# sulaimanvesal/PointCloudUDA

Hardware: AMD Instinct MI355X
Metric: adversarial train-step images/sec (seg+3 discr) at 256x256 (higher is better)
Workload: dtype bf16x3 MFMA (split-bf16, fp32 accumulate; fp32 storage); 1 GPU; MS-CMRSeg full UDA: UNet(PointNet head) + d1 + d2 + d4, 256x256x1, 4 classes; per_gpu_batch=32, global_batch=32, precision=bf16x3, parallelism=dp1, ranks_in_group=1, collective=none, streams=discriminators concurrent, d_target_forward=replayed from the adversarial pass of the same step, launch=eager (256 host cores for this rank)

## Files before the change

include/pcuda_hip.h:

```cpp
#ifndef PCUDA_HIP_H
#define PCUDA_HIP_H

#include <stddef.h>
#include <stdint.h>

#ifdef __cplusplus
extern "C" {
#endif

#define PCUDA_OK 0
#define PCUDA_E_BADARG (-1)
#define PCUDA_E_UNSUPPORTED (-2)
#define PCUDA_E_LAUNCH (-3)
#define PCUDA_E_WORKSPACE (-4)

#define PCUDA_PREC_BF16X3 0
#define PCUDA_PREC_BF16 1

typedef void* pcuda_stream_t;

#define PCUDA_ABI_VERSION 5
int pcuda_version(void);
size_t pcuda_abi_struct_size(int which);
int pcuda_device_count(void);
// ... 2 lines not shown
long long pcuda_launch_count(int reset);
long long pcuda_fallback_count(void);
const char* pcuda_last_kernel(void);
int pcuda_clock_probe(unsigned long long* out2_dev, float* sink_dev, int iters, pcuda_stream_t s);

#define PCUDA_FAM_CONV_FWD 0
#define PCUDA_FAM_CONV_WGRAD 1
#define PCUDA_FAM_POINTWISE 2
#define PCUDA_FAM_DENSE_F32 3
#define PCUDA_FAM_COUNT 4
int pcuda_prof_enable(int on);
int pcuda_prof_reset(void);
int pcuda_prof_read(int family, double* ms, double* work, long long* launches);
int pcuda_prof_dump(const char* path);
int pcuda_debug_read_clocks(unsigned long long* out8);

typedef struct pcuda_conv_geom {
  int n;
  int cin, cout;
  int in_h, in_w;
  int out_h, out_w;
  int k, stride, pad, dil;
  int in_up;
} pcuda_conv_geom;

typedef struct pcuda_src {
  const float* p1; long long sn1, sc1; const float* scale1; const float* shift1;
  const float* p2; long long sn2, sc2; const float* scale2; const float* shift2;
  int c1;
} pcuda_src;
typedef struct pcuda_dst {
  float* p1; long long sn1, sc1;
  float* p2; long long sn2, sc2;
  int c1;
} pcuda_dst;

size_t pcuda_conv2d_packed_fwd_bytes(const pcuda_conv_geom* g, int prec);
size_t pcuda_conv2d_packed_dgrad_bytes(const pcuda_conv_geom* g, int prec);
int pcuda_conv2d_pack_fwd(const pcuda_conv_geom* g, int prec, const float* w, void* packed, pcuda_stream_t s);
int pcuda_conv2d_pack_dgrad(const pcuda_conv_geom* g, int prec, const float* w, void* packed, pcuda_stream_t s);
int pcuda_conv2d_pack_all(const pcuda_conv_geom* g, int prec, const float* w, void* packed_fwd, void* packed_dgrad,
                          pcuda_stream_t s);
size_t pcuda_conv2d_pack_job_bytes(void);
int pcuda_conv2d_pack_jobs_fill(const pcuda_conv_geom* g, int prec, const float* w, void* packed_fwd, void* packed_dgrad,
                                void* host_jobs, int max_jobs, int* job_blocks);
int pcuda_conv2d_pack_table(const void* dev_jobs, const int* dev_first_block, int njobs, int total_blocks, pcuda_stream_t s);

int pcuda_conv2d_d1_forward_ok(const pcuda_conv_geom* g);
int pcuda_conv2d_fwd_tiles(const pcuda_conv_geom* g, int prec);
int pcuda_conv2d_forward(const pcuda_conv_geom* g, int prec, const pcuda_src* x, const void* packed_w,
                         const float* bias, float slope, const pcuda_dst* y, float* bn_partials,
                         pcuda_stream_t s);
int pcuda_conv2d_dgrad(const pcuda_conv_geom* g, int prec, const pcuda_src* dy, const void* packed_w_dgrad,
                       const pcuda_dst* dx, int accumulate, pcuda_stream_t s);
int pcuda_conv2d_dgrad_tiles(const pcuda_conv_geom* g, int prec);
int pcuda_conv2d_dgrad_bnred(const pcuda_conv_geom* g, int prec, const pcuda_src* dy, const void* packed_w_dgrad,
                             const pcuda_dst* dx, int accumulate, const float* a, long long a_sn, long long a_sc,
                             const float* mean, const float* invstd, float* red_partials, pcuda_stream_t s);
int pcuda_conv2d_dgrad_lrelu(const pcuda_conv_geom* g, int prec, const pcuda_src* dy, const void* packed_w_dgrad,
                             const pcuda_dst* dx, const float* a, long long a_sn, long long a_sc, float slope,
                             pcuda_stream_t s);
int pcuda_conv2d_dgrad_fold(const pcuda_conv_geom* g, int prec, const pcuda_src* dy, const void* packed_w_dgrad,
                            const pcuda_dst* dx_half, const float* a, long long a_sn, long long a_sc, const float* mean,
                            const float* invstd, float* red_partials, pcuda_stream_t s);
size_t pcuda_conv2d_wgrad_workspace_size(const pcuda_conv_geom* g);
int pcuda_conv2d_wgrad(const pcuda_conv_geom* g, int prec, const pcuda_src* x, const float* dy,
                       long long dy_sn, long long dy_sc, float* dw, float* db, int accumulate,
                       void* workspace, size_t workspace_bytes, pcuda_stream_t s);

#define PCUDA_REDUCE_MAX_JOBS 56
typedef struct {
  const float* partial;
  long long numel;
  float* dw;
  const float* db_partial;
  long long nb;
  float* db;
  int ksplit, nkg, accumulate, ntaps;
} pcuda_reduce_job;
int pcuda_conv2d_wgrad_partial(const pcuda_conv_geom* g, int prec, const pcuda_src* x, const float* dy,
                               long long dy_sn, long long dy_sc, float* dw, float* db, int accumulate,
                               void* workspace, size_t workspace_bytes, pcuda_reduce_job* job, pcuda_stream_t s);
int pcuda_wgrad_reduce_batch(const pcuda_reduce_job* host_jobs, int njobs, pcuda_stream_t s);

int pcuda_bn_finalize(const float* partials, int ntiles, int c, long long count, const float* gamma,
                      const float* beta, float eps, float momentum, float* running_mean, float* running_var,
                      float* mean, float* invstd, float* scale, float* shift, pcuda_stream_t s);
int pcuda_bn_stats(const float* a, long long sn, long long sc, int n, int c, long long hw,
                   float* partials, int* ntiles, pcuda_stream_t s);
#define PCUDA_BN_APPLY_RELU 1
#define PCUDA_BN_APPLY_FMA 2
int pcuda_bn_apply(const float* a, long long a_sn, long long a_sc, const float* scale, const float* shift,
                   int flags, float* y, long long y_sn, long long y_sc, int n, int c, long long hw,
                   pcuda_stream_t s);
int pcuda_bn_bwd_reduce(const float* dy, long long dy_sn, long long dy_sc, const float* dy2, long long dy2_sn,
                        long long dy2_sc, const float* a, long long a_sn, long long a_sc, const float* mean,
                        const float* invstd, const float* scale, const float* shift, int post_relu, int n, int c,
                        long long hw, float* red, int* ntiles, pcuda_stream_t s);
int pcuda_bn_bwd_finalize(const float* red, int ntiles, int c, long long count, const float* gamma,
                          const float* invstd, const float* mean, float* dgamma, float* dbeta, int accumulate,
                          float* coef , pcuda_stream_t s);
int pcuda_bn_bwd_apply(const float* dy, long long dy_sn, long long dy_sc, const float* dy2, long long dy2_sn,
                       long long dy2_sc, const float* a, long long a_sn, long long a_sc, const float* coef,
                       const float* scale, const float* shift, int post_relu, float act_slope, float* dz,
                       long long dz_sn, long long dz_sc, int n, int c, long long hw, pcuda_stream_t s);
int pcuda_lrelu_bwd(const float* dy, long long dy_sn, long long dy_sc, const float* dy2, long long dy2_sn,
                    long long dy2_sc, const float* a, long long a_sn, long long a_sc, float slope, float* dz,
                    long long dz_sn, long long dz_sc, int n, int c, long long hw, pcuda_stream_t s);
int pcuda_channel_sum(const float* dz, long long sn, long long sc, int n, int c, long long hw, float* db,
                      int accumulate, float* workspace, size_t workspace_bytes, pcuda_stream_t s);

int pcuda_maxpool2_fwd(const float* x, long long x_sn, long long x_sc, const float* scale, const float* shift,
                       float* y, long long y_sn, long long y_sc, uint8_t* idx, int n, int c, int h, int w,
                       pcuda_stream_t s);
int pcuda_maxpool2_bwd(const float* dy, long long dy_sn, long long dy_sc, const float* dy2, long long dy2_sn,
                       long long dy2_sc, const uint8_t* idx, float* dx, long long dx_sn, long long dx_sc,
                       int accumulate, int n, int c, int h, int w, pcuda_stream_t s);
typedef struct pcuda_pooled {
  const float* g; long long g_sn, g_sc;
  const float* g2; long long g2_sn, g2_sc;
  const uint8_t* idx;
  int h, w;
} pcuda_pooled;
int pcuda_bn_bwd_reduce_pooled(const pcuda_pooled* pool, const float* dy, long long dy_sn, long long dy_sc, const float* a,
                               long long a_sn, long long a_sc, const float* mean, const float* invstd, int n, int c,
                               float* red, int* ntiles, pcuda_stream_t s);
int pcuda_bn_bwd_apply_pooled(const pcuda_pooled* pool, const float* dy, long long dy_sn, long long dy_sc, const float* a,
                              long long a_sn, long long a_sc, const float* coef, float act_slope, float* dz, long long dz_sn,
                              long long dz_sc, int n, int c, pcuda_stream_t s);
int pcuda_lrelu_bwd_pooled(const pcuda_pooled* pool, const float* dy, long long dy_sn, long long dy_sc, const float* a,
                           long long a_sn, long long a_sc, float slope, float* dz, long long dz_sn, long long dz_sc, int n,
                           int c, pcuda_stream_t s);
int pcuda_upsample2_bwd(const float* dy, long long dy_sn, long long dy_sc, float* dx, long long dx_sn,
                        long long dx_sc, int accumulate, int n, int c, int h, int w, pcuda_stream_t s);
int pcuda_upsample2_bwd_bnred(const float* dy, long long dy_sn, long long dy_sc, float* dx, long long dx_sn,
                              long long dx_sc, int accumulate, const float* a, long long a_sn, long long a_sc,
                              const float* mean, const float* invstd, float* red, int* ntiles, int n, int c, int h, int w,
                              pcuda_stream_t s);
int pcuda_bilinear_fwd(const float* x, long long x_sn, long long x_sc, int n, int c, int h, int w, float* y, int oh,
                       int ow, pcuda_stream_t s);
int pcuda_bilinear_bwd(const float* dy, int n, int c, int oh, int ow, float* dx, long long dx_sn, long long dx_sc,
                       int h, int w, pcuda_stream_t s);
int pcuda_unfold_taps(const float* x, long long x_sn, long long x_sc, int n, int c, int h, int w, int k, int stride,
                      int pad, int dil, float* u, int oh, int ow, pcuda_stream_t s);
int pcuda_add4(const float* a, const float* b, const float* c, const float* d, float* y, long long numel,
               pcuda_stream_t s);
int pcuda_mul(const float* a, const float* b, float* y, long long numel, pcuda_stream_t s);

#define PCUDA_ACT_SIGMOID 0
#define PCUDA_ACT_SOFTMAX 1
int pcuda_entropy_fwd(const float* logits, int mode, float norm, float* ent, float* prob, int n, int c,
                      long long hw, pcuda_stream_t s);
int pcuda_entropy_bwd(const float* logits, int mode, float norm, const float* dent, const float* dprob,
                      float* dlogits, int accumulate, int n, int c, long long hw, pcuda_stream_t s);
int pcuda_entropy_bwd2(const float* logits, int mode, float norm, const float* dent, const float* dprob, const float* dmean,
                       float* dlogits, int accumulate, int n, int c, long long hw, pcuda_stream_t s);
size_t pcuda_sum_all_workspace_size(void);
int pcuda_sum_all(const float* x, long long numel, double scale, float* out, void* workspace, size_t workspace_bytes,
                  pcuda_stream_t s);
size_t pcuda_seg_loss_workspace_size(int n, int c, long long hw);
int pcuda_seg_loss_fwd(const float* logits, const uint8_t* onehot, int mode, int n, int c, long long hw,
                       float* out2, void* workspace, size_t workspace_bytes, pcuda_stream_t s);
int pcuda_seg_loss_bwd(const float* logits, const uint8_t* onehot, int mode, int n, int c, long long hw,
                       const float* g_main, const float* g_jac, float* dlogits, const void* workspace,
                       pcuda_stream_t s);
int pcuda_bce_const_fwd(const float* x, long long numel, float label, float* loss, float* acc, pcuda_stream_t s);
// ... 251 lines not shown
```

pointcloududa_amd/_lib.py:

```python
from __future__ import annotations

import ctypes as C
import os

_HERE = os.path.dirname(os.path.abspath(__file__))
LIB_PATH = os.environ.get("PCUDA_LIB") or os.path.join(_HERE, "lib", "libpcuda_hip.so")

PREC_BF16X3, PREC_BF16 = 0, 1
ACT_SIGMOID, ACT_SOFTMAX = 0, 1
OV_DICE_CLASS, OV_DICE_SAMPLE = 1, 2
FAM_CONV_FWD, FAM_CONV_WGRAD, FAM_POINTWISE, FAM_DENSE_F32 = 0, 1, 2, 3

c_f32p = C.c_void_p
i32, i64, f32, f64, vp, sz = C.c_int, C.c_longlong, C.c_float, C.c_double, C.c_void_p, C.c_size_t


class ConvGeom(C.Structure):
    _fields_ = [("n", i32), ("cin", i32), ("cout", i32), ("in_h", i32), ("in_w", i32), ("out_h", i32),
                ("out_w", i32), ("k", i32), ("stride", i32), ("pad", i32), ("dil", i32), ("in_up", i32)]


class ReduceJob(C.Structure):
    _fields_ = [("partial", C.c_void_p), ("numel", C.c_longlong), ("dw", C.c_void_p), ("db_partial", C.c_void_p),
                ("nb", C.c_longlong), ("db", C.c_void_p), ("ksplit", C.c_int), ("nkg", C.c_int), ("accumulate", C.c_int),
                ("ntaps", C.c_int)]


class Src(C.Structure):
    _fields_ = [("p1", vp), ("sn1", i64), ("sc1", i64), ("scale1", vp), ("shift1", vp),
                ("p2", vp), ("sn2", i64), ("sc2", i64), ("scale2", vp), ("shift2", vp), ("c1", i32)]


class Dst(C.Structure):
    _fields_ = [("p1", vp), ("sn1", i64), ("sc1", i64), ("p2", vp), ("sn2", i64), ("sc2", i64), ("c1", i32)]


class Pooled(C.Structure):
    _fields_ = [("g", vp), ("g_sn", i64), ("g_sc", i64), ("g2", vp), ("g2_sn", i64), ("g2_sc", i64), ("idx", vp),
                ("h", i32), ("w", i32)]


_PROTOS = {
    "pcuda_version": (i32, []),
    "pcuda_device_count": (i32, []),
    "pcuda_last_error": (C.c_char_p, []),
    "pcuda_build_hash": (C.c_char_p, []),
    "pcuda_launch_count": (i64, [i32]),
    "pcuda_fallback_count": (i64, []),
    "pcuda_abi_struct_size": (sz, [i32]),
    "pcuda_last_kernel": (C.c_char_p, []),
    "pcuda_clock_probe": (i32, [vp, vp, i32, vp]),
    "pcuda_prof_enable": (i32, [i32]),
    "pcuda_prof_reset": (i32, []),
    "pcuda_prof_read": (i32, [i32, C.POINTER(C.c_double), C.POINTER(C.c_double), C.POINTER(i64)]),
    "pcuda_prof_dump": (i32, [C.c_char_p]),
    "pcuda_debug_read_clocks": (i32, [vp]),
    "pcuda_conv2d_packed_fwd_bytes": (sz, [C.POINTER(ConvGeom), i32]),
    "pcuda_conv2d_packed_dgrad_bytes": (sz, [C.POINTER(ConvGeom), i32]),
    "pcuda_conv2d_pack_fwd": (i32, [C.POINTER(ConvGeom), i32, vp, vp, vp]),
    "pcuda_conv2d_pack_all": (i32, [C.POINTER(ConvGeom), i32, vp, vp, vp, vp]),
    "pcuda_conv2d_pack_dgrad": (i32, [C.POINTER(ConvGeom), i32, vp, vp, vp]),
    "pcuda_conv2d_pack_job_bytes": (sz, []),
    "pcuda_conv2d_pack_jobs_fill": (i32, [C.POINTER(ConvGeom), i32, vp, vp, vp, vp, i32, C.POINTER(i32)]),
    "pcuda_conv2d_pack_table": (i32, [vp, vp, i32, i32, vp]),
    "pcuda_conv2d_fwd_tiles": (i32, [C.POINTER(ConvGeom), i32]),
    "pcuda_conv2d_forward": (i32, [C.POINTER(ConvGeom), i32, C.POINTER(Src), vp, vp, f32, C.POINTER(Dst), vp, vp]),
    "pcuda_conv2d_d1_forward_ok": (i32, [C.POINTER(ConvGeom)]),
    "pcuda_conv2d_dgrad": (i32, [C.POINTER(ConvGeom), i32, C.POINTER(Src), vp, C.POINTER(Dst), i32, vp]),
    "pcuda_conv2d_dgrad_tiles": (i32, [C.POINTER(ConvGeom), i32]),
    "pcuda_conv2d_dgrad_bnred": (i32, [C.POINTER(ConvGeom), i32, C.POINTER(Src), vp, C.POINTER(Dst), i32, vp, i64, i64, vp,
                                       vp, vp, vp]),
    "pcuda_conv2d_dgrad_fold": (i32, [C.POINTER(ConvGeom), i32, C.POINTER(Src), vp, C.POINTER(Dst), vp, i64, i64, vp, vp, vp, vp]),
    "pcuda_conv2d_dgrad_lrelu": (i32, [C.POINTER(ConvGeom), i32, C.POINTER(Src), vp, C.POINTER(Dst), vp, i64, i64, f32, vp]),
    "pcuda_conv2d_wgrad_workspace_size": (sz, [C.POINTER(ConvGeom)]),
    "pcuda_conv2d_wgrad": (i32, [C.POINTER(ConvGeom), i32, C.POINTER(Src), vp, i64, i64, vp, vp, i32, vp, sz, vp]),
    "pcuda_conv2d_wgrad_partial": (i32, [C.POINTER(ConvGeom), i32, C.POINTER(Src), vp, i64, i64, vp, vp, i32, vp, sz,
                                         C.POINTER(ReduceJob), vp]),
    "pcuda_wgrad_reduce_batch": (i32, [C.POINTER(ReduceJob), i32, vp]),
    "pcuda_bn_finalize": (i32, [vp, i32, i32, i64, vp, vp, f32, f32, vp, vp, vp, vp, vp, vp, vp]),
    "pcuda_bn_stats": (i32, [vp, i64, i64, i32, i32, i64, vp, C.POINTER(i32), vp]),
    "pcuda_bn_apply": (i32, [vp, i64, i64, vp, vp, i32, vp, i64, i64, i32, i32, i64, vp]),
    "pcuda_bn_bwd_reduce": (i32, [vp, i64, i64, vp, i64, i64, vp, i64, i64, vp, vp, vp, vp, i32, i32, i32, i64, vp,
                                  C.POINTER(i32), vp]),
    "pcuda_bn_bwd_finalize": (i32, [vp, i32, i32, i64, vp, vp, vp, vp, vp, i32, vp, vp]),
    "pcuda_bn_bwd_apply": (i32, [vp, i64, i64, vp, i64, i64, vp, i64, i64, vp, vp, vp, i32, f32, vp, i64, i64, i32,
                                 i32, i64, vp]),
    "pcuda_lrelu_bwd": (i32, [vp, i64, i64, vp, i64, i64, vp, i64, i64, f32, vp, i64, i64, i32, i32, i64, vp]),
    "pcuda_channel_sum": (i32, [vp, i64, i64, i32, i32, i64, vp, i32, vp, sz, vp]),
    "pcuda_maxpool2_fwd": (i32, [vp, i64, i64, vp, vp, vp, i64, i64, vp, i32, i32, i32, i32, vp]),
    "pcuda_maxpool2_bwd": (i32, [vp, i64, i64, vp, i64, i64, vp, vp, i64, i64, i32, i32, i32, i32, i32, vp]),
    "pcuda_bn_bwd_reduce_pooled": (i32, [C.POINTER(Pooled), vp, i64, i64, vp, i64, i64, vp, vp, i32, i32, vp, C.POINTER(i32), vp]),
    "pcuda_bn_bwd_apply_pooled": (i32, [C.POINTER(Pooled), vp, i64, i64, vp, i64, i64, vp, f32, vp, i64, i64, i32, i32, vp]),
    "pcuda_lrelu_bwd_pooled": (i32, [C.POINTER(Pooled), vp, i64, i64, vp, i64, i64, f32, vp, i64, i64, i32, i32, vp]),
    "pcuda_upsample2_bwd": (i32, [vp, i64, i64, vp, i64, i64, i32, i32, i32, i32, i32, vp]),
    "pcuda_upsample2_bwd_bnred": (i32, [vp, i64, i64, vp, i64, i64, i32, vp, i64, i64, vp, vp, vp, C.POINTER(i32), i32, i32,
                                        i32, i32, vp]),
    "pcuda_bilinear_fwd": (i32, [vp, i64, i64, i32, i32, i32, i32, vp, i32, i32, vp]),
    "pcuda_bilinear_bwd": (i32, [vp, i32, i32, i32, i32, vp, i64, i64, i32, i32, vp]),
    "pcuda_unfold_taps": (i32, [vp, i64, i64, i32, i32, i32, i32, i32, i32, i32, i32, vp, i32, i32, vp]),
    "pcuda_add4": (i32, [vp, vp, vp, vp, vp, i64, vp]),
    "pcuda_mul": (i32, [vp, vp, vp, i64, vp]),
    "pcuda_entropy_fwd": (i32, [vp, i32, f32, vp, vp, i32, i32, i64, vp]),
    "pcuda_entropy_bwd": (i32, [vp, i32, f32, vp, vp, vp, i32, i32, i32, i64, vp]),
    "pcuda_entropy_bwd2": (i32, [vp, i32, f32, vp, vp, vp, vp, i32, i32, i32, i64, vp]),
    "pcuda_sum_all_workspace_size": (sz, []),
    "pcuda_sum_all": (i32, [vp, i64, C.c_double, vp, vp, sz, vp]),
    "pcuda_seg_loss_workspace_size": (sz, [i32, i32, i64]),
    "pcuda_seg_loss_fwd": (i32, [vp, vp, i32, i32, i32, i64, vp, vp, sz, vp]),
    "pcuda_seg_loss_bwd": (i32, [vp, vp, i32, i32, i32, i64, vp, vp, vp, vp, vp]),
    "pcuda_jaccard_workspace_size": (sz, [i32]),
    "pcuda_jaccard_fwd": (i32, [vp, vp, i32, i32, i32, i64, f32, vp, vp, sz, vp]),
    "pcuda_jaccard_bwd": (i32, [vp, i32, i32, i32, i64, f32, vp, vp, vp, vp]),
    "pcuda_seg_loss_ov_workspace_size": (sz, [i32, i32, i64, i32]),
    "pcuda_seg_loss_ov_fwd": (i32, [vp, vp, i32, i32, C.c_double, i32, i32, i64, vp, vp, sz, vp]),
    "pcuda_seg_loss_ov_bwd": (i32, [vp, vp, i32, i32, i32, i32, i64, vp, vp, vp, vp, sz, vp]),
    "pcuda_dice_workspace_size": (sz, [i32, i32, i64, i32]),
    "pcuda_dice_fwd": (i32, [vp, vp, i32, i32, i32, i64, i32, f32, vp, vp, sz, vp]),
    "pcuda_dice_bwd": (i32, [vp, i32, i32, i32, i64, i32, vp, vp, vp, sz, vp]),
    "pcuda_dice_labels_workspace_size": (sz, [i32, i32, i64]),
    "pcuda_dice_labels_fwd": (i32, [vp, vp, i32, i32, i32, i64, f32, vp, vp, vp, sz, vp]),
    "pcuda_dice_labels_bwd": (i32, [vp, vp, i32, i32, i32, i64, vp, vp, vp, sz, vp]),
    "pcuda_bce_const_fwd": (i32, [vp, i64, f32, vp, vp, vp]),
    "pcuda_bce_const_bwd": (i32, [vp, i64, f32, vp, f32, vp, vp]),
    "pcuda_nn_loss_workspace_floats": (sz, [i32, i32]),
    "pcuda_nn_loss_fwd": (i32, [vp, vp, i32, i32, vp, vp, vp, vp]),
    "pcuda_nn_loss_bwd": (i32, [vp, vp, i32, i32, vp, vp, vp, vp, vp]),
    "pcuda_dice_metric": (i32, [vp, vp, i32, i32, i64, vp, vp, sz, vp]),
    "pcuda_assemble_batch": (i32, [vp, vp, i32, i32, i32, i32, i32, i32, vp, vp, vp]),
    "pcuda_minmax_workspace_size": (sz, []),
    "pcuda_minmax": (i32, [vp, i64, vp, vp, sz, vp]),
    "pcuda_augment_assemble": (i32, [vp, i32, vp, i32, i32, i32, i32, i32, i32, vp, vp, vp, i32, vp, vp, vp, vp, vp, vp, vp]),
    "pcuda_quantize_u8": (i32, [vp, i64, vp, vp, vp]),
    "pcuda_augment_assemble_dequant": (i32, [vp, vp, i32, i32, i32, i32, i32, i32, vp, vp, vp, vp, vp, vp, vp, vp, vp, vp]),
    "pcuda_photometric_workspace_size": (sz, [i32, i32, i32, i32]),
    "pcuda_photometric": (i32, [vp, vp, i32, i32, i32, i32, i32, vp, vp, vp, vp, vp, sz, vp]),
    "pcuda_geometric_workspace_size": (sz, [i32, i32, i32, i32, i32]),
    "pcuda_geometric": (i32, [vp, vp, vp, vp, i32, i32, i32, i32, i32, vp, vp, vp, vp, vp, sz, vp]),
    "pcuda_geometric_cubic": (i32, [vp, vp, vp, vp, i32, i32, i32, i32, i32, vp, vp, vp, vp, vp, sz, vp]),
    "pcuda_stylize_workspace_size": (sz, [i32, i32, i32, i32]),
    "pcuda_stylize": (i32, [vp, vp, i32, i32, i32, i32, i32, vp, vp, vp, vp, vp, vp, sz, vp]),
    "pcuda_stylize_connect_workspace_size": (sz, [i32, i32, i32, i32]),
    "pcuda_stylize_connect": (i32, [vp, vp, i32, i32, i32, i32, i32, vp, vp, vp, vp, vp, vp, sz, vp]),
    "pcuda_stylize_scaled_workspace_size": (sz, [i32, i32, i32, i32]),
    "pcuda_stylize_scaled": (i32, [vp, vp, i32, i32, i32, i32, i32, vp, vp, vp, vp, vp, vp, sz, vp]),
    "pcuda_crop_pad_workspace_size": (sz, [i32, i32, i32, i32]),
    "pcuda_crop_pad": (i32, [vp, vp, vp, vp, i32, i32, i32, i32, vp, vp, vp, sz, vp]),
    "pcuda_match_hist_workspace_size": (sz, [i32, i32, i32, i32, i32]),
    "pcuda_match_hist": (i32, [vp, vp, i32, i32, i32, i32, i32, vp, vp, vp, i32, vp, sz, vp]),
    "pcuda_hist_bank_size": (sz, [i32, i32, i32, i32, i32]),
    "pcuda_hist_bank_workspace_size": (sz, [i32, i32, i32, i32, i32]),
    "pcuda_hist_bank_build": (i32, [vp, i32, i32, i32, i32, i32, vp, sz, vp, vp, sz, vp]),
    "pcuda_match_hist_bank_workspace_size": (sz, [i32, i32, i32, i32, i32]),
    "pcuda_match_hist_bank": (i32, [vp, vp, i32, i32, i32, i32, i32, vp, i32, i32, i32, vp, vp, sz, vp]),
    "pcuda_fourier_bank_size": (sz, [i32, i32, i32]),
    "pcuda_fourier_bank_workspace_size": (sz, [i32, i32, i32, i32, i32]),
    "pcuda_fourier_bank_build": (i32, [vp, i32, i32, i32, i32, i32, i32, vp, sz, vp, sz, vp]),
    "pcuda_fourier_adapt_workspace_size": (sz, [i32, i32, i32, i32, i32]),
    "pcuda_fourier_adapt": (i32, [vp, vp, i32, i32, i32, i32, i32, vp, i32, i32, vp, vp, i32, f64, f64, vp, sz, vp]),
    "pcuda_clahe_workspace_size": (sz, [i32, i32, i32]),
    "pcuda_clahe": (i32, [vp, vp, i32, i32, i32, f64, i32, i32, i32, vp, sz, vp]),
    "pcuda_rescale_resize_crop_u8_workspace_size": (sz, []),
# ... 109 lines not shown
```

pointcloududa_amd/csrc/conv_wgrad.hip:

```cpp
#include "conv_igemm.h"
#include "conv_host.h"

struct ReduceJobs {
  int n;
  int first_block[PCUDA_REDUCE_MAX_JOBS + 1];
  pcuda_reduce_job j[PCUDA_REDUCE_MAX_JOBS];
};

__global__ __launch_bounds__(1024) void wgrad_reduce_batch_kernel(const ReduceJobs jobs) {
  __shared__ float sh[16][64];
  int lo = 0, hi = jobs.n - 1;
  while (lo < hi) {
    const int mid = (lo + hi + 1) >> 1;
    if (jobs.first_block[mid] <= (int)blockIdx.x) lo = mid; else hi = mid - 1;
  }
  const pcuda_reduce_job& jb = jobs.j[lo];
  const float* partial = jb.partial;
  long long numel = jb.numel;
  float* dw = jb.dw;
  int ntaps = jb.ntaps;
  const int ksplit = jb.ksplit, nkg = jb.nkg;
  const int lane = threadIdx.x & 63, kg = threadIdx.x >> 6;
  const long long nblk_w = (numel + 63) / 64;
  long long blk = (int)blockIdx.x - jobs.first_block[lo];
  if (blk >= nblk_w) { blk -= nblk_w; partial = jb.db_partial; numel = jb.nb; dw = jb.db; ntaps = 1; }
  const long long i = blk * 64 + lane;
  float s = 0.f;
  if (i < numel && kg < nkg) {
    int k = kg;
    for (; k + 7 * nkg < ksplit; k += 8 * nkg) {
      float v[8];
#pragma unroll
      for (int u = 0; u < 8; ++u) v[u] = partial[(long long)(k + u * nkg) * numel + i];
#pragma unroll
      for (int u = 0; u < 8; ++u) s += v[u];
    }
    for (; k < ksplit; k += nkg) s += partial[(long long)k * numel + i];
  }
  sh[kg][lane] = s;
  __syncthreads();
  if (kg == 0 && i < numel) {
    float t = 0.f;
    for (int q = 0; q < nkg; ++q) t += sh[q][lane];
    long long o = i;
    if (ntaps > 1) {
      const long long cc = numel / ntaps;
      const long long tt = i / cc, r = i - tt * cc;
      o = r * ntaps + tt;
    }
    dw[o] = jb.accumulate ? dw[o] + t : t;
  }
}

static int reduce_blocks(const pcuda_reduce_job& jb) { return cdiv(jb.numel, 64) + (jb.db ? cdiv(jb.nb, 64) : 0); }

static int launch_reduce_jobs(const ReduceJobs& jobs, int threads, hipStream_t s) {
  hipLaunchKernelGGL(wgrad_reduce_batch_kernel, dim3(jobs.first_block[jobs.n]), dim3(threads), 0, s, jobs);
  PCUDA_CHECK_LAUNCH("wgrad_reduce_batch_kernel");
  return PCUDA_OK;
}

static pcuda_reduce_job reduce_job(const float* partial, long long numel, int ksplit, float* dw, int accumulate, int ntaps,
                                   const float* db_partial, long long nb, float* db) {
  pcuda_reduce_job jb;
  memset(&jb, 0, sizeof(jb));
  jb.partial = partial; jb.numel = numel; jb.ksplit = ksplit; jb.dw = dw; jb.accumulate = accumulate; jb.ntaps = ntaps;
  jb.db_partial = db_partial; jb.nb = db ? nb : 0; jb.db = db;
  jb.nkg = 1;
  while (jb.nkg < 16 && jb.nkg * 2 <= ksplit) jb.nkg <<= 1;
  return jb;
}

static int launch_reduce_job(const pcuda_reduce_job& jb, hipStream_t s) {
  ReduceJobs jobs;
  jobs.n = 1;
  jobs.j[0] = jb;
  jobs.first_block[0] = 0;
  jobs.first_block[1] = reduce_blocks(jb);
  return launch_reduce_jobs(jobs, 64 * jb.nkg, s);
}
int launch_wgrad_reduce(const float* partial, long long numel, int ksplit, float* dw, int accumulate, int ntaps,
                        const float* db_partial, long long nb, float* db, hipStream_t s) {
  return launch_reduce_job(reduce_job(partial, numel, ksplit, dw, accumulate, ntaps, db_partial, nb, db), s);
}

WgradSlabs wgrad_slabs(const WgradCall& c, int slices, int ntaps) {
  WgradSlabs sl;
  sl.welems = (long long)c.g->cout * c.g->cin * c.g->k * c.g->k;
  sl.partial = (float*)c.workspace;
  sl.db_partial = c.db ? sl.partial + (size_t)slices * sl.welems : nullptr;
  sl.slices = slices; sl.ntaps = ntaps;
  return sl;
}

int wgrad_finish(const WgradCall& c, const WgradSlabs& sl) {
  const pcuda_reduce_job jb = reduce_job(sl.partial, sl.welems, sl.slices, c.dw, c.accumulate, sl.ntaps, sl.db_partial, c.g->cout, c.db);
  if (!c.defer) return launch_reduce_job(jb, c.s);
  *c.defer = jb;
  return PCUDA_OK;
}

extern "C" int pcuda_wgrad_reduce_batch(const pcuda_reduce_job* host_jobs, int njobs, pcuda_stream_t s) {
  if (!host_jobs || njobs < 0) PCUDA_FAIL(PCUDA_E_BADARG, "wgrad_reduce_batch: bad arguments");
  int done = 0;
  while (done < njobs) {
    ReduceJobs jobs;
    jobs.n = 0;
    int blocks = 0;
    for (; done < njobs && jobs.n < PCUDA_REDUCE_MAX_JOBS; ++done) {
      const pcuda_reduce_job& jb = host_jobs[done];
      if (jb.ksplit <= 0) continue;
      if (!jb.partial || !jb.dw || jb.numel <= 0 || jb.nkg < 1 || jb.nkg > 16 || (jb.db && !jb.db_partial))
        PCUDA_FAIL(PCUDA_E_BADARG, "wgrad_reduce_batch: bad job %d", done);
      jobs.first_block[jobs.n] = blocks;
      jobs.j[jobs.n++] = jb;
      blocks += reduce_blocks(jb);
    }
    if (jobs.n == 0) break;
    jobs.first_block[jobs.n] = blocks;
    ProfScope prof(PCUDA_FAM_POINTWISE, 0.0, (hipStream_t)s, "wgrad reduce batch");
    const int rc = launch_reduce_jobs(jobs, 1024, (hipStream_t)s);
    if (rc) return rc;
  }
  return PCUDA_OK;
}

namespace {

struct WgradPlan {
  int co_blks, co_tile, n_co_tiles, n_chunks, tap_groups, taps_per_group, tw, th, tiles_x, tiles_y, ksplit;
  int ih_t, iw_t;
};

struct TileSpan {
  long long halo, clipped;
};
TileSpan tile_span(const pcuda_conv_geom* g, long long ih, long long iw) {
  return {ih * iw, (ih < g->in_h ? ih : g->in_h) * (iw < g->in_w ? iw : g->in_w) + 1};
}
size_t stage_lds(long long x_pixels, int co_tile, size_t mul) {
  return (size_t)x_pixels * IG_REC_BYTES * mul + (size_t)co_tile * WG_ZROW * mul;
}

struct WgradStage {
  bool clamp;
  int x_cap;
  size_t lds;
};
WgradStage wgrad_stage(const WgradPlan& w, const pcuda_conv_geom* g, size_t mul) {
  const TileSpan t = tile_span(g, w.ih_t, w.iw_t);
  WgradStage st;
  st.clamp = t.clipped * 2 <= t.halo || stage_lds(t.halo, w.co_tile, mul) > (size_t)LDS_HARD;
  st.x_cap = (int)(st.clamp ? t.clipped : t.halo);
  st.lds = stage_lds(st.x_cap, w.co_tile, mul);
  return st;
}

WgradPlan plan_wgrad(const pcuda_conv_geom* g) {
  WgradPlan w;
  w.co_blks = ig_co_blks(g->cout);
  w.co_tile = 32 * w.co_blks;
  w.n_co_tiles = cdiv(g->cout, w.co_tile);
  w.n_chunks = cdiv(g->cin, 32);
  const int ntaps = g->k * g->k;
  w.tap_groups = ntaps <= 16 ? 1 : cdiv(ntaps, 9);
  w.taps_per_group = cdiv(ntaps, w.tap_groups);
  const int span = (g->k - 1) * g->dil;
  {
    int cand[16];
    const int nc = tile_width_candidates(g->out_w, 128, cand);
    long long best_key = -1;
    w.tw = 32; w.th = 4;
    for (int ci = 0; ci < nc; ++ci) {
      const int tw = cand[ci], th = 128 / tw;
      if (th < 1) continue;
      const TileSpan t = tile_span(g, (th - 1) * g->stride + span + 1, (tw - 1) * g->stride + span + 1);
      const long long cap = t.halo < t.clipped ? t.halo : t.clipped;
      if (stage_lds(cap, w.co_tile, 2) > (size_t)LDS_HARD) continue;
      const long long staged = (t.clipped * 2 <= t.halo) ? t.clipped : t.halo;
      const long long key = ((long long)cdiv(g->out_w, tw) * cdiv(g->out_h, th) << 24) + (staged > 768 ? (1ll << 22) : 0) +
                            ((tw & 31) ? (1ll << 20) : 0) + t.halo;
      if (best_key < 0 || key < best_key) { best_key = key; w.tw = tw; w.th = th; }
    }
  }
  const int TW = w.tw, TH = w.th;
  w.tiles_x = cdiv(g->out_w, TW);
  w.tiles_y = cdiv(g->out_h, TH);
  w.ih_t = (TH - 1) * g->stride + span + 1;
  w.iw_t = (TW - 1) * g->stride + span + 1;
  const long long ntiles = (long long)g->n * w.tiles_x * w.tiles_y;
  const int base = w.n_co_tiles * w.n_chunks * w.tap_groups;
  static const int tgt32 = env_knob("PCUDA_WG_BLOCKS32", 768);
  static const int tgt64 = env_knob("PCUDA_WG_BLOCKS64", 1024);
  static const int tgt1 = env_knob("PCUDA_WG_BLOCKS1", 256);
  const bool one_per_cu = wgrad_stage(w, g, 2).lds > (size_t)LDS_HARD / 2;
  long long ks = (one_per_cu ? tgt1 : (w.co_blks == 1 ? tgt32 : tgt64)) / base;
  if (ks < 1) ks = 1;
  if (ks > ntiles) ks = ntiles;
  const long long welems = (long long)g->cout * g->cin * ntaps;
  while (ks > 1 && ks * welems * 4 > (64ll << 20)) ks >>= 1;
  if (ks >= 8) ks &= ~7ll;
  w.ksplit = (int)ks;
  return w;
}

int wgrad_prefetch(const WgradCall& c, const WgradPlan& w, int x_cap) {
// ... 133 lines not shown
```

pointcloududa_amd/csrc/dense.hip:

```cpp
#include "common.h"

struct GemmParams {
  const float* a; long long a_sb, a_si, a_sl;
  const float* b; long long b_sb, b_sl, b_sj;
  float* c; long long c_sb, c_si, c_sj;
  const float* bias;
  int m, n, k, accumulate;
};

#define GT 32
__global__ __launch_bounds__(256) void gemm_kernel(const GemmParams p) {
  __shared__ float As[GT][GT + 1], Bs[GT][GT + 1];
  const int bz = blockIdx.z;
  const float* A = p.a + bz * p.a_sb;
  const float* B = p.b + bz * p.b_sb;
  float* C = p.c + bz * p.c_sb;
  const int i0 = blockIdx.y * GT, j0 = blockIdx.x * GT;
  const int tj = threadIdx.x & 31, ti = threadIdx.x >> 5;
  float acc[4] = {0.f, 0.f, 0.f, 0.f};
  for (int l0 = 0; l0 < p.k; l0 += GT) {
    for (int e = threadIdx.x; e < GT * GT; e += 256) {
      const int r = e >> 5, cc = e & 31;
      int ia, la;
      if (p.a_sl == 1) { ia = r; la = cc; } else { ia = cc; la = r; }
      As[ia][la] = (i0 + ia < p.m && l0 + la < p.k) ? A[(i0 + ia) * p.a_si + (l0 + la) * p.a_sl] : 0.f;
      int lb, jb;
      if (p.b_sj == 1) { lb = r; jb = cc; } else { lb = cc; jb = r; }
      Bs[lb][jb] = (l0 + lb < p.k && j0 + jb < p.n) ? B[(l0 + lb) * p.b_sl + (j0 + jb) * p.b_sj] : 0.f;
    }
    __syncthreads();
#pragma unroll 8
    for (int l = 0; l < GT; ++l) {
      const float bv = Bs[l][tj];
#pragma unroll
      for (int q = 0; q < 4; ++q) acc[q] += As[ti * 4 + q][l] * bv;
    }
    __syncthreads();
  }
  const int j = j0 + tj;
  if (j < p.n) {
    const float bj = p.bias ? p.bias[j] : 0.f;
#pragma unroll
    for (int q = 0; q < 4; ++q) {
      const int i = i0 + ti * 4 + q;
      if (i < p.m) {
        float* dst = C + i * p.c_si + j * p.c_sj;
        const float v = acc[q] + bj;
        *dst = p.accumulate ? *dst + v : v;
      }
    }
  }
}

#define SK_COLS 8
#define SK_WAVES 16
__global__ __launch_bounds__(64 * SK_WAVES) void gemm_skinny_kernel(const GemmParams p) {
  __shared__ float red[SK_WAVES][64][SK_COLS];
  const int lane = threadIdx.x & 63, wv = threadIdx.x >> 6;
  const int j0 = blockIdx.x * SK_COLS;
  const int i = min(lane, p.m - 1);
  const float* arow = p.a + (long long)i * p.a_si;
  const int kq = (p.k + SK_WAVES - 1) / SK_WAVES, l_lo = wv * kq, l_hi = min(p.k, l_lo + kq);
  float acc[SK_COLS];
#pragma unroll
  for (int c = 0; c < SK_COLS; ++c) acc[c] = 0.f;
  const float* bcol[SK_COLS];
#pragma unroll
  for (int c = 0; c < SK_COLS; ++c) bcol[c] = p.b + (long long)min(j0 + c, p.n - 1) * p.b_sj;
#pragma unroll 4
  for (int l = l_lo; l < l_hi; ++l) {
    const float av = arow[(long long)l * p.a_sl];
#pragma unroll
    for (int c = 0; c < SK_COLS; ++c) acc[c] = fmaf(av, bcol[c][(long long)l * p.b_sl], acc[c]);
  }
#pragma unroll
  for (int c = 0; c < SK_COLS; ++c) red[wv][lane][c] = acc[c];
  __syncthreads();
  for (int e = threadIdx.x; e < 64 * SK_COLS; e += 64 * SK_WAVES) {
    const int r = e / SK_COLS, c = e - r * SK_COLS, j = j0 + c;
    if (r < p.m && j < p.n) {
      float v = 0.f;
#pragma unroll
      for (int q = 0; q < SK_WAVES; ++q) v += red[q][r][c];
      v += p.bias ? p.bias[j] : 0.f;
      float* dst = p.c + (long long)r * p.c_si + (long long)j * p.c_sj;
      *dst = p.accumulate ? *dst + v : v;
    }
  }
}


__global__ __launch_bounds__(256) void colsum_kernel(const float* __restrict__ dy, int m, int n, float* db,
                                                     int accumulate, int cp) {
  __shared__ float sh[256];
  const int rparts = 256 / cp;
  const int c = threadIdx.x % cp, rp = threadIdx.x / cp;
  const int j = blockIdx.x * cp + c;
  float s = 0.f;
  if (j < n)
    for (int i = rp; i < m; i += rparts) s += dy[(long long)i * n + j];
  sh[threadIdx.x] = s;
  __syncthreads();
  for (int half = rparts >> 1; half > 0; half >>= 1) {
    if (rp < half) sh[threadIdx.x] += sh[threadIdx.x + half * cp];
    __syncthreads();
  }
  if (rp == 0 && j < n) db[j] = accumulate ? db[j] + sh[c] : sh[c];
}

__global__ void splitk_reduce_kernel(const float* __restrict__ part, long long numel, int ksplit,
                                     float* __restrict__ out, int accumulate) {
  for (long long i = blockIdx.x * (long long)blockDim.x + threadIdx.x; i < numel;
       i += (long long)gridDim.x * blockDim.x) {
    float s = 0.f;
    for (int k = 0; k < ksplit; ++k) s += part[(long long)k * numel + i];
    out[i] = accumulate ? out[i] + s : s;
  }
}

__global__ __launch_bounds__(256) void max_points_fwd_kernel(const float* __restrict__ x, int rows, int l,
                                                             float* __restrict__ y, int* __restrict__ idx) {
  const int row = blockIdx.x * 4 + (threadIdx.x >> 6), lane = threadIdx.x & 63;
  if (row >= rows) return;
  const float* p = x + (long long)row * l;
  float best = -INFINITY;
  int bi = 0x7fffffff;
  for (int i = lane; i < l; i += 64) {
    const float v = p[i];
    if (v > best) { best = v; bi = i; }
  }
#pragma unroll
  for (int o = 32; o > 0; o >>= 1) {
    const float ov = __shfl_xor(best, o, 64);
    const int oi = __shfl_xor(bi, o, 64);
    if (ov > best || (ov == best && oi < bi)) { best = ov; bi = oi; }
  }
  if (lane == 0) { y[row] = best; idx[row] = bi; }
}

__global__ __launch_bounds__(256) void max_points_bwd_kernel(const float* __restrict__ dy, const int* __restrict__ idx,
                                                             int rows, int l, float* __restrict__ dx) {
  const long long total = (long long)rows * l;
  for (long long e = blockIdx.x * 256ll + threadIdx.x; e < total; e += 256ll * gridDim.x) {
    const int row = (int)(e / l), i = (int)(e - (long long)row * l);
    dx[e] = (idx[row] == i) ? dy[row] : 0.f;
  }
}

namespace {
int launch_gemm(const GemmParams& p, int batch, hipStream_t s) {
  if (p.m <= 0 || p.n <= 0 || p.k <= 0 || batch <= 0) PCUDA_FAIL(PCUDA_E_BADARG, "gemm: bad dims");
  if (batch == 1 && p.m <= 64 && p.k >= 64) {
    hipLaunchKernelGGL(gemm_skinny_kernel, dim3(cdiv(p.n, SK_COLS)), dim3(64 * SK_WAVES), 0, s, p);
    PCUDA_CHECK_LAUNCH("gemm_skinny_kernel");
    return PCUDA_OK;
  }
  dim3 grid(cdiv(p.n, GT), cdiv(p.m, GT), batch);
  hipLaunchKernelGGL(gemm_kernel, grid, dim3(256), 0, s, p);
  PCUDA_CHECK_LAUNCH("gemm_kernel");
  return PCUDA_OK;
}
}

extern "C" int pcuda_linear_fwd(const float* x, const float* w, const float* b, float* y, int m, int k, int n,
                                pcuda_stream_t s) {
  if (!x || !w || !y) PCUDA_FAIL(PCUDA_E_BADARG, "linear_fwd: null pointer");
  GemmParams p = {x, 0, k, 1, w, 0, 1, k, y, 0, n, 1, b, m, n, k, 0};
  return launch_gemm(p, 1, (hipStream_t)s);
}

extern "C" int pcuda_linear_bwd_x(const float* dy, const float* w, float* dx, int m, int k, int n, int accumulate,
                                  pcuda_stream_t s) {
  if (!dy || !w || !dx) PCUDA_FAIL(PCUDA_E_BADARG, "linear_bwd_x: null pointer");
  GemmParams p = {dy, 0, n, 1, w, 0, k, 1, dx, 0, k, 1, nullptr, m, k, n, accumulate};
  return launch_gemm(p, 1, (hipStream_t)s);
}

extern "C" size_t pcuda_linear_bwd_w_workspace_size(int m, int k, int n) {
  const long long out_elems = (long long)n * k;
  if (m >= 2048 && out_elems <= 65536) {
    int ks = m / 256;
    if (ks > 64) ks = 64;
    return (size_t)(ks + 1) * out_elems * sizeof(float);
  }
  return 0;
}

extern "C" int pcuda_linear_bwd_w(const float* dy, const float* x, float* dw, float* db, int m, int k, int n,
                                  int accumulate, void* workspace, size_t workspace_bytes, pcuda_stream_t s) {
  if (!dy || !x || !dw) PCUDA_FAIL(PCUDA_E_BADARG, "linear_bwd_w: null pointer");
  const long long out_elems = (long long)n * k;
  const size_t need = pcuda_linear_bwd_w_workspace_size(m, k, n);
  int rc;
  if (need > 0 && workspace && workspace_bytes >= need) {
    float* slab = (float*)workspace;
    int ks = m / 256;
    if (ks > 64) ks = 64;
    const int mk = (m + ks - 1) / ks;
    const int full = m / mk;
    GemmParams pb = {dy, (long long)mk * n, 1, n, x, (long long)mk * k, k, 1, slab, out_elems, k, 1, nullptr, n, k, mk, 0};
    rc = launch_gemm(pb, full, (hipStream_t)s);
    if (rc) return rc;
    int nsl = full;
    if (m - full * mk > 0) {
      GemmParams pt = {dy + (long long)full * mk * n, 0, 1, n, x + (long long)full * mk * k, 0, k, 1,
                       slab + (long long)full * out_elems, 0, k, 1, nullptr, n, k, m - full * mk, 0};
      rc = launch_gemm(pt, 1, (hipStream_t)s);
      if (rc) return rc;
      ++nsl;
    }
    hipLaunchKernelGGL(splitk_reduce_kernel, dim3(cdiv(out_elems, 256)), dim3(256), 0, (hipStream_t)s,
                       (const float*)slab, out_elems, nsl, dw, accumulate);
    PCUDA_CHECK_LAUNCH("splitk_reduce_kernel");
  } else {
    GemmParams p = {dy, 0, 1, n, x, 0, k, 1, dw, 0, k, 1, nullptr, n, k, m, accumulate};
    rc = launch_gemm(p, 1, (hipStream_t)s);
    if (rc) return rc;
  }
  if (db) {
    int cp = 1;
    while (cp < n && cp < 64) cp <<= 1;
    hipLaunchKernelGGL(colsum_kernel, dim3(cdiv(n, cp)), dim3(256), 0, (hipStream_t)s, dy, m, n, db, accumulate, cp);
    PCUDA_CHECK_LAUNCH("colsum_kernel");
  }
  return PCUDA_OK;
}

extern "C" int pcuda_bmm(const float* a, const float* bmat, float* c, int batch, int m, int k, int n, int ta, int tb,
                         int accumulate, pcuda_stream_t s) {
  if (!a || !bmat || !c) PCUDA_FAIL(PCUDA_E_BADARG, "bmm: null pointer");
  GemmParams p;
  p.a = a; p.a_sb = (long long)m * k; p.a_si = ta ? 1 : k; p.a_sl = ta ? m : 1;
  p.b = bmat; p.b_sb = (long long)k * n; p.b_sl = tb ? 1 : n; p.b_sj = tb ? k : 1;
  p.c = c; p.c_sb = (long long)m * n; p.c_si = n; p.c_sj = 1;
  p.bias = nullptr; p.m = m; p.n = n; p.k = k; p.accumulate = accumulate;
  return launch_gemm(p, batch, (hipStream_t)s);
}
// ... 18 lines not shown
```

Measured before the change: 786.8 img/s.

## Vectorize wgrad reduce, add LDS-staged skinny GEMM, unroll split-K reduce

```diff
diff --git a/include/pcuda_hip.h b/include/pcuda_hip.h
--- a/include/pcuda_hip.h
+++ b/include/pcuda_hip.h
@@ -108,6 +108,7 @@
                                long long dy_sn, long long dy_sc, float* dw, float* db, int accumulate,
                                void* workspace, size_t workspace_bytes, pcuda_reduce_job* job, pcuda_stream_t s);
 int pcuda_wgrad_reduce_batch(const pcuda_reduce_job* host_jobs, int njobs, pcuda_stream_t s);
+int pcuda_wgrad_reduce_bounds(const pcuda_reduce_job* job, long long* out4);
 
 int pcuda_bn_finalize(const float* partials, int ntiles, int c, long long count, const float* gamma,
                       const float* beta, float eps, float momentum, float* running_mean, float* running_var,
diff --git a/pointcloududa_amd/_lib.py b/pointcloududa_amd/_lib.py
--- a/pointcloududa_amd/_lib.py
+++ b/pointcloududa_amd/_lib.py
@@ -77,6 +77,7 @@
     "pcuda_conv2d_wgrad_partial": (i32, [C.POINTER(ConvGeom), i32, C.POINTER(Src), vp, i64, i64, vp, vp, i32, vp, sz,
                                          C.POINTER(ReduceJob), vp]),
     "pcuda_wgrad_reduce_batch": (i32, [C.POINTER(ReduceJob), i32, vp]),
+    "pcuda_wgrad_reduce_bounds": (i32, [C.POINTER(ReduceJob), C.POINTER(i64)]),
     "pcuda_bn_finalize": (i32, [vp, i32, i32, i64, vp, vp, f32, f32, vp, vp, vp, vp, vp, vp, vp]),
     "pcuda_bn_stats": (i32, [vp, i64, i64, i32, i32, i64, vp, C.POINTER(i32), vp]),
     "pcuda_bn_apply": (i32, [vp, i64, i64, vp, vp, i32, vp, i64, i64, i32, i32, i64, vp]),
diff --git a/pointcloududa_amd/csrc/conv_wgrad.hip b/pointcloududa_amd/csrc/conv_wgrad.hip
--- a/pointcloududa_amd/csrc/conv_wgrad.hip
+++ b/pointcloududa_amd/csrc/conv_wgrad.hip
@@ -1,5 +1,94 @@
 #include "conv_igemm.h"
 #include "conv_host.h"
+
+#ifndef PCUDA_REDUCE_FILL
+#define PCUDA_REDUCE_FILL 128
+#endif
+#define REDUCE_VEC 4
+#define REDUCE_INFLIGHT 8
+
+__host__ __device__ inline int reduce_vec(long long numel) { return numel >= 64ll * REDUCE_VEC * PCUDA_REDUCE_FILL ? REDUCE_VEC : 1; }
+__host__ __device__ inline long long reduce_span_blocks(long long numel) {
+  const long long per = 64ll * reduce_vec(numel);
+  return (numel + per - 1) / per;
+}
+struct ReduceLane {
+  long long i0, ld0;
+  int cnt, skip;
+};
+__host__ __device__ inline ReduceLane reduce_lane(long long numel, int vec, long long blk, int lane) {
+  ReduceLane ln;
+  ln.i0 = (blk * 64 + lane) * vec;
+  const long long left = numel - ln.i0;
+  ln.cnt = left <= 0 ? 0 : (left < vec ? (int)left : vec);
+  ln.skip = ln.cnt ? vec - ln.cnt : 0;
+  ln.ld0 = ln.i0 - ln.skip;
+  return ln;
+}
+__host__ __device__ inline long long reduce_src_index(long long numel, int k, long long i) { return (long long)k * numel + i; }
+__host__ __device__ inline long long reduce_dst_index(long long numel, int ntaps, long long i) {
+  if (ntaps <= 1) return i;
+  const long long cc = numel / ntaps;
+  const long long tt = i / cc, r = i - tt * cc;
+  return r * ntaps + tt;
+}
+
+template <int V, class Mem>
+__host__ __device__ inline void reduce_kgroup(Mem& mem, long long numel, int ksplit, int nkg, int kg, long long ld0, float (&s)[V]) {
+  int k = kg;
+  for (; k + (REDUCE_INFLIGHT - 1) * nkg < ksplit; k += REDUCE_INFLIGHT * nkg) {
+    float v[REDUCE_INFLIGHT][V];
+#pragma unroll
+    for (int u = 0; u < REDUCE_INFLIGHT; ++u) mem.template load<V>(reduce_src_index(numel, k + u * nkg, ld0), v[u]);
+#pragma unroll
+    for (int u = 0; u < REDUCE_INFLIGHT; ++u)
+#pragma unroll
+      for (int c = 0; c < V; ++c) s[c] += v[u][c];
+  }
+  if (k < ksplit) {
+    float v[REDUCE_INFLIGHT - 1][V];
+#pragma unroll
+    for (int u = 0; u < REDUCE_INFLIGHT - 1; ++u) {
+#pragma unroll
+      for (int c = 0; c < V; ++c) v[u][c] = 0.f;
+      if (k + u * nkg < ksplit) mem.template load<V>(reduce_src_index(numel, k + u * nkg, ld0), v[u]);
+    }
+#pragma unroll
+    for (int u = 0; u < REDUCE_INFLIGHT - 1; ++u)
+      if (k + u * nkg < ksplit) {
+#pragma unroll
+        for (int c = 0; c < V; ++c) s[c] += v[u][c];
+      }
+  }
+}
+
+typedef float f32x4_a4 __attribute__((ext_vector_type(4), aligned(4)));
+struct ReduceDeviceMem {
+  const float* p;
+  template <int V>
+  __device__ __forceinline__ void load(long long idx, float (&v)[V]) const {
+    if constexpr (V == 4) {
+      const f32x4_a4 t = *(const f32x4_a4*)(p + idx);
+      v[0] = t[0]; v[1] = t[1]; v[2] = t[2]; v[3] = t[3];
+    } else {
+      static_assert(V == 1, "one 16-byte or one 4-byte load");
+      v[0] = p[idx];
+    }
+  }
+};
+struct ReduceModelMem {
+  long long hi = -1, lo = 0;
+  template <int V>
+  void load(long long idx, float (&v)[V]) {
+    for (int c = 0; c < V; ++c) v[c] = 0.f;
+    touch(idx);
+    touch(idx + V - 1);
+  }
+  void touch(long long idx) {
+    if (idx > hi) hi = idx;
+    if (idx < lo) lo = idx;
+  }
+};
 
 struct ReduceJobs {
   int n;
@@ -7,52 +96,61 @@
   pcuda_reduce_job j[PCUDA_REDUCE_MAX_JOBS];
 };
 
+struct ReduceSpan {
+  const float* partial;
+  float* out;
+  long long numel, blk;
+  int ntaps;
+};
+__host__ __device__ inline long long reduce_blocks(const pcuda_reduce_job& jb) {
+  return reduce_span_blocks(jb.numel) + (jb.db ? reduce_span_blocks(jb.nb) : 0);
+}
+__host__ __device__ inline ReduceSpan reduce_span(const pcuda_reduce_job& jb, long long blk) {
+  const long long nblk_w = reduce_span_blocks(jb.numel);
+  if (blk < nblk_w) return {jb.partial, jb.dw, jb.numel, blk, jb.ntaps};
+  return {jb.db_partial, jb.db, jb.nb, blk - nblk_w, 1};
+}
+
+template <int V>
+__device__ __forceinline__ void reduce_span_run(float (&sh)[16][64 * REDUCE_VEC], const ReduceSpan& sp, int ksplit, int nkg, int accumulate) {
+  const int lane = threadIdx.x & 63, kg = threadIdx.x >> 6;
+  const ReduceLane ln = reduce_lane(sp.numel, V, sp.blk, lane);
+  if (kg < nkg) {
+    float s[V];
+#pragma unroll
+    for (int c = 0; c < V; ++c) s[c] = 0.f;
+    if (ln.cnt) {
+      ReduceDeviceMem mem = {sp.partial};
+      reduce_kgroup<V>(mem, sp.numel, ksplit, nkg, kg, ln.ld0, s);
+    }
+#pragma unroll
+    for (int c = 0; c < V; ++c)
+      if (c >= ln.skip) sh[kg][lane * V + c - ln.skip] = s[c];
+  }
+  __syncthreads();
+  for (int e = threadIdx.x; e < 64 * V; e += blockDim.x) {
+    const long long i = sp.blk * (64 * V) + e;
+    if (i < sp.numel) {
+      float t = 0.f;
+      for (int q = 0; q < nkg; ++q) t += sh[q][e];
+      const long long o = reduce_dst_index(sp.numel, sp.ntaps, i);
+      sp.out[o] = accumulate ? sp.out[o] + t : t;
+    }
+  }
+}
+
 __global__ __launch_bounds__(1024) void wgrad_reduce_batch_kernel(const ReduceJobs jobs) {
-  __shared__ float sh[16][64];
+  __shared__ float sh[16][64 * REDUCE_VEC];
   int lo = 0, hi = jobs.n - 1;
   while (lo < hi) {
     const int mid = (lo + hi + 1) >> 1;
     if (jobs.first_block[mid] <= (int)blockIdx.x) lo = mid; else hi = mid - 1;
   }
   const pcuda_reduce_job& jb = jobs.j[lo];
-  const float* partial = jb.partial;
-  long long numel = jb.numel;
-  float* dw = jb.dw;
-  int ntaps = jb.ntaps;
-  const int ksplit = jb.ksplit, nkg = jb.nkg;
-  const int lane = threadIdx.x & 63, kg = threadIdx.x >> 6;
-  const long long nblk_w = (numel + 63) / 64;
-  long long blk = (int)blockIdx.x - jobs.first_block[lo];
-  if (blk >= nblk_w) { blk -= nblk_w; partial = jb.db_partial; numel = jb.nb; dw = jb.db; ntaps = 1; }
-  const long long i = blk * 64 + lane;
-  float s = 0.f;
-  if (i < numel && kg < nkg) {
-    int k = kg;
-    for (; k + 7 * nkg < ksplit; k += 8 * nkg) {
-      float v[8];
-#pragma unroll
-      for (int u = 0; u < 8; ++u) v[u] = partial[(long long)(k + u * nkg) * numel + i];
-#pragma unroll
-      for (int u = 0; u < 8; ++u) s += v[u];
-    }
-    for (; k < ksplit; k += nkg) s += partial[(long long)k * numel + i];
-  }
-  sh[kg][lane] = s;
-  __syncthreads();
-  if (kg == 0 && i < numel) {
-    float t = 0.f;
-    for (int q = 0; q < nkg; ++q) t += sh[q][lane];
-    long long o = i;
-    if (ntaps > 1) {
-      const long long cc = numel / ntaps;
-      const long long tt = i / cc, r = i - tt * cc;
-      o = r * ntaps + tt;
-    }
-    dw[o] = jb.accumulate ? dw[o] + t : t;
-  }
-}
-
-static int reduce_blocks(const pcuda_reduce_job& jb) { return cdiv(jb.numel, 64) + (jb.db ? cdiv(jb.nb, 64) : 0); }
+  const ReduceSpan sp = reduce_span(jb, (int)blockIdx.x - jobs.first_block[lo]);
+  if (reduce_vec(sp.numel) == 1) reduce_span_run<1>(sh, sp, jb.ksplit, jb.nkg, jb.accumulate);
+  else reduce_span_run<REDUCE_VEC>(sh, sp, jb.ksplit, jb.nkg, jb.accumulate);
+}
 
 static int launch_reduce_jobs(const ReduceJobs& jobs, int threads, hipStream_t s) {
   hipLaunchKernelGGL(wgrad_reduce_batch_kernel, dim3(jobs.first_block[jobs.n]), dim3(threads), 0, s, jobs);
@@ -110,7 +208,7 @@
     for (; done < njobs && jobs.n < PCUDA_REDUCE_MAX_JOBS; ++done) {
       const pcuda_reduce_job& jb = host_jobs[done];
       if (jb.ksplit <= 0) continue;
-      if (!jb.partial || !jb.dw || jb.numel <= 0 || jb.nkg < 1 || jb.nkg > 16 || (jb.db && !jb.db_partial))
+      if (!jb.partial || !jb.dw || jb.numel <= 0 || jb.numel < jb.ntaps || jb.nkg < 1 || jb.nkg > 16 || (jb.db && !jb.db_partial))
         PCUDA_FAIL(PCUDA_E_BADARG, "wgrad_reduce_batch: bad job %d", done);
       jobs.first_block[jobs.n] = blocks;
       jobs.j[jobs.n++] = jb;
@@ -122,6 +220,40 @@
     const int rc = launch_reduce_jobs(jobs, 1024, (hipStream_t)s);
     if (rc) return rc;
   }
+  return PCUDA_OK;
+}
+
+template <int V>
+static void reduce_model_lane(ReduceModelMem& src, const ReduceSpan& sp, const pcuda_reduce_job& jb, int lane) {
+  const ReduceLane ln = reduce_lane(sp.numel, V, sp.blk, lane);
+  if (!ln.cnt) return;
+  for (int kg = 0; kg < jb.nkg; ++kg) {
+    float s[V] = {};
+    reduce_kgroup<V>(src, sp.numel, jb.ksplit, jb.nkg, kg, ln.ld0, s);
+  }
+}
+
+extern "C" int pcuda_wgrad_reduce_bounds(const pcuda_reduce_job* job, long long* out4) {
+  if (!job || !out4) PCUDA_FAIL(PCUDA_E_BADARG, "wgrad_reduce_bounds: null pointer");
+  const pcuda_reduce_job& jb = *job;
+  if (jb.numel <= 0 || jb.nb < 0 || jb.ksplit < 1 || jb.nkg < 1 || jb.nkg > 16 || (jb.db && !jb.db_partial) ||
+      jb.numel < jb.ntaps)
+    PCUDA_FAIL(PCUDA_E_BADARG, "wgrad_reduce_bounds: bad job");
+  ReduceModelMem mem[4];
+  const long long nblk = reduce_blocks(jb), nblk_w = reduce_span_blocks(jb.numel);
+  for (long long blk = 0; blk < nblk; ++blk) {
+    const ReduceSpan sp = reduce_span(jb, blk);
+    const int bias = blk >= nblk_w ? 1 : 0, vec = reduce_vec(sp.numel);
+    for (int lane = 0; lane < 64; ++lane) {
+      if (vec == 1) reduce_model_lane<1>(mem[bias], sp, jb, lane);
+      else reduce_model_lane<REDUCE_VEC>(mem[bias], sp, jb, lane);
+    }
+    for (int e = 0; e < 64 * vec; ++e) {
+      const long long i = sp.blk * (64 * vec) + e;
+      if (i < sp.numel) mem[2 + bias].touch(reduce_dst_index(sp.numel, sp.ntaps, i));
+    }
+  }
+  for (int b = 0; b < 4; ++b) out4[b] = mem[b].lo < 0 ? 0x7fffffffffffffffll : mem[b].hi;
   return PCUDA_OK;
 }
 
diff --git a/pointcloududa_amd/csrc/dense.hip b/pointcloududa_amd/csrc/dense.hip
--- a/pointcloududa_amd/csrc/dense.hip
+++ b/pointcloududa_amd/csrc/dense.hip
@@ -89,6 +89,111 @@
   }
 }
 
+typedef float f32x4_a4 __attribute__((ext_vector_type(4), aligned(4)));
+__host__ __device__ inline int sk_pitch(int m) { return ((m + 7) & ~7) + 2; }
+static size_t sk_lds_bytes(int m, int kc) {
+  const size_t stage = (size_t)SK_WAVES * kc * (sk_pitch(m) + SK_COLS), red = (size_t)SK_WAVES * 64 * SK_COLS;
+  return (stage > red ? stage : red) * sizeof(float);
+}
+
+template <int KC>
+__global__ __launch_bounds__(64 * SK_WAVES) void gemm_skinny_staged_kernel(const GemmParams p) {
+  extern __shared__ __attribute__((aligned(16))) float sk_lds[];
+  constexpr int NA = KC / 4, NB = KC / SK_COLS;
+  const int lane = threadIdx.x & 63, wv = threadIdx.x >> 6;
+  const int j0 = blockIdx.x * SK_COLS;
+  const int pitch = sk_pitch(p.m);
+  float* As = sk_lds + wv * KC * pitch;
+  float* Bs = sk_lds + SK_WAVES * KC * pitch + wv * KC * SK_COLS;
+  const int kq = (p.k + SK_WAVES - 1) / SK_WAVES, l_lo = wv * kq, l_hi = min(p.k, l_lo + kq);
+  const int nch = (kq + KC - 1) / KC;
+  f32x4 ra[NA];
+  float rb[NB];
+  auto b_item = [&](int e, int& c, int& li) {
+    if (p.b_sl == 1) { c = e / KC; li = e % KC; } else { c = e % SK_COLS; li = e / SK_COLS; }
+  };
+  auto fetch = [&](int l0) {
+#pragma unroll
+    for (int j = 0; j < NA; ++j) {
+      const int it = j * 64 + lane, row = it / NA, l = l0 + (it % NA) * 4, nv = l_hi - l;
+      ra[j] = f32x4{0.f, 0.f, 0.f, 0.f};
+      if (row < p.m && nv > 0) {
+        const float* q = p.a + (long long)row * p.a_si + l;
+        if (nv >= 4) {
+          ra[j] = *(const f32x4_a4*)q;
+        } else {
+          ra[j][0] = q[0];
+          if (nv > 1) ra[j][1] = q[1];
+          if (nv > 2) ra[j][2] = q[2];
+        }
+      }
+    }
+#pragma unroll
+    for (int j = 0; j < NB; ++j) {
+      int c, li;
+      b_item(j * 64 + lane, c, li);
+      rb[j] = 0.f;
+      if (l0 + li < l_hi) rb[j] = p.b[(long long)(l0 + li) * p.b_sl + (long long)min(j0 + c, p.n - 1) * p.b_sj];
+    }
+  };
+  float acc[SK_COLS];
+#pragma unroll
+  for (int c = 0; c < SK_COLS; ++c) acc[c] = 0.f;
+  const int rr = min(lane, p.m - 1);
+  fetch(l_lo);
+  for (int ch = 0; ch < nch; ++ch) {
+    const int l0 = l_lo + ch * KC;
+#pragma unroll
+    for (int j = 0; j < NA; ++j) {
+      const int it = j * 64 + lane, row = it / NA, lq = (it % NA) * 4;
+      if (row < p.m) {
+#pragma unroll
+        for (int e = 0; e < 4; ++e) As[(lq + e) * pitch + row] = ra[j][e];
+      }
+    }
+#pragma unroll
+    for (int j = 0; j < NB; ++j) {
+      int c, li;
+      b_item(j * 64 + lane, c, li);
+      Bs[li * SK_COLS + c] = rb[j];
+    }
+    __syncthreads();
+    if (ch + 1 < nch) fetch(l0 + KC);
+    const int nl = min(KC, l_hi - l0);
+    auto step = [&](int li) {
+      const float av = As[li * pitch + rr];
+      const f32x4 b0 = *(const f32x4*)(Bs + li * SK_COLS), b1 = *(const f32x4*)(Bs + li * SK_COLS + 4);
+#pragma unroll
+      for (int c = 0; c < 4; ++c) {
+        acc[c] = fmaf(av, b0[c], acc[c]);
+        acc[c + 4] = fmaf(av, b1[c], acc[c + 4]);
+      }
+    };
+    if (nl == KC) {
+#pragma unroll 4
+      for (int li = 0; li < KC; ++li) step(li);
+    } else {
+      for (int li = 0; li < nl; ++li) step(li);
+    }
+    __syncthreads();
+  }
+  float* red = sk_lds;
+#pragma unroll
+  for (int c = 0; c < SK_COLS; ++c) red[(wv * 64 + lane) * SK_COLS + c] = acc[c];
+  __syncthreads();
+  for (int e = threadIdx.x; e < 64 * SK_COLS; e += 64 * SK_WAVES) {
+    const int r = e / SK_COLS, c = e - r * SK_COLS, j = j0 + c;
+    if (r < p.m && j < p.n) {
+      float v = 0.f;
+#pragma unroll
+      for (int q = 0; q < SK_WAVES; ++q) v += red[(q * 64 + r) * SK_COLS + c];
+      v += p.bias ? p.bias[j] : 0.f;
+      float* dst = p.c + (long long)r * p.c_si + (long long)j * p.c_sj;
+      *dst = p.accumulate ? *dst + v : v;
+    }
+  }
+}
+
 
 __global__ __launch_bounds__(256) void colsum_kernel(const float* __restrict__ dy, int m, int n, float* db,
                                                      int accumulate, int cp) {
@@ -113,8 +218,35 @@
   for (long long i = blockIdx.x * (long long)blockDim.x + threadIdx.x; i < numel;
        i += (long long)gridDim.x * blockDim.x) {
     float s = 0.f;
-    for (int k = 0; k < ksplit; ++k) s += part[(long long)k * numel + i];
-    out[i] = accumulate ? out[i] + s : s;
+    int k = 0;
+    for (; k + 7 < ksplit; k += 8) {
+      float v[8];
+      const float* q[8];
+#pragma unroll
+      for (int u = 0; u < 8; ++u) { q[u] = part + ((long long)(k + u) * numel + i); v[u] = *q[u]; }
+#pragma unroll
+      for (int u = 0; u < 8; ++u) s += v[u];
+#pragma unroll
+      for (int u = 0; u < 8; ++u) PCUDA_KEEP(q[u]);
+    }
+    if (k < ksplit) {
+      float v[7];
+      const float* q[7];
+#pragma unroll
+      for (int u = 0; u < 7; ++u) {
+        v[u] = 0.f;
+        q[u] = part + ((long long)min(k + u, ksplit - 1) * numel + i);
+        if (k + u < ksplit) v[u] = *q[u];
+      }
+#pragma unroll
+      for (int u = 0; u < 7; ++u)
+        if (k + u < ksplit) s += v[u];
+#pragma unroll
+      for (int u = 0; u < 7; ++u) PCUDA_KEEP(q[u]);
+    }
+    float* o = out + i;
+    *o = accumulate ? *o + s : s;
+    PCUDA_KEEP(o);
   }
 }
 
@@ -151,8 +283,17 @@
 int launch_gemm(const GemmParams& p, int batch, hipStream_t s) {
   if (p.m <= 0 || p.n <= 0 || p.k <= 0 || batch <= 0) PCUDA_FAIL(PCUDA_E_BADARG, "gemm: bad dims");
   if (batch == 1 && p.m <= 64 && p.k >= 64) {
-    hipLaunchKernelGGL(gemm_skinny_kernel, dim3(cdiv(p.n, SK_COLS)), dim3(64 * SK_WAVES), 0, s, p);
-    PCUDA_CHECK_LAUNCH("gemm_skinny_kernel");
+    const dim3 grid(cdiv(p.n, SK_COLS)), block(64 * SK_WAVES);
+    if (p.a_sl != 1) {
+      hipLaunchKernelGGL(gemm_skinny_kernel, grid, block, 0, s, p);
+      PCUDA_CHECK_LAUNCH("gemm_skinny_kernel");
+    } else if (sk_lds_bytes(p.m, 16) <= (size_t)(64 << 10)) {
+      hipLaunchKernelGGL(gemm_skinny_staged_kernel<16>, grid, block, sk_lds_bytes(p.m, 16), s, p);
+      PCUDA_CHECK_LAUNCH("gemm_skinny_staged_kernel");
+    } else {
+      hipLaunchKernelGGL(gemm_skinny_staged_kernel<8>, grid, block, sk_lds_bytes(p.m, 8), s, p);
+      PCUDA_CHECK_LAUNCH("gemm_skinny_staged_kernel");
+    }
     return PCUDA_OK;
   }
   dim3 grid(cdiv(p.n, GT), cdiv(p.m, GT), batch);
```

After: 791.0 img/s (median of 6 runs). Within noise of the previous version (+0.5%).
